# k-sheridan/mantis

Measured on AMD Instinct MI355X. Metric: poses/sec + p50 per-frame latency, 1280x720 4-cam batch, higher is better.
Workload: dtype f64; 1 GPU; config3: 4-cam 1280x720 rig, shared map, full mantis3 path per camera + joint rig Gauss-Newton; cams_per_rig=4, contexts_per_gpu=6, landmarks=720, parallelism=rig-data-parallel x1

## Files before the change

include/mantis.h:

```cpp
#ifndef MANTIS_H
#define MANTIS_H
#include <stddef.h>
#include <stdint.h>

#ifdef __cplusplus
extern "C" {
#endif

#define MANTIS_ABI_VERSION 5

typedef enum mantis_status {
  MANTIS_OK = 0,
  MANTIS_ERR_ARG = 1,
  MANTIS_ERR_DEVICE = 2,
  MANTIS_ERR_OOM = 3,
  MANTIS_ERR_CAPACITY = 4,
  MANTIS_ERR_STATE = 5,
  MANTIS_ERR_COMM = 6
} mantis_status;

typedef enum mantis_reason {
  MANTIS_PUBLISHED = 0,
  MANTIS_NO_QUADS = 1,
  MANTIS_NO_HYPS = 2,
// ... 147 lines not shown
mantis_status mantis_gn_accumulate(void* ctx, const double* T_w_b, const double* T_base_cam, int32_t n_cams,
                                   const double* obs, int32_t n_obs, double* acc28);
mantis_status mantis_gn_solve(const double* acc28, double lambda, double* T_w_b, double* delta6);

mantis_status mantis_comm_unique_id(void* id128);
mantis_status mantis_comm_init(void* ctx, const void* id128, int32_t nranks, int32_t rank);
mantis_status mantis_comm_info(void* ctx, int32_t* nranks, int32_t* rank);
mantis_status mantis_gn_allreduce(void* ctx, double* acc28);

typedef struct mantis_synth_cam {
  double fx, fy, cx, cy;
  double k[4];
  double R_wc[9];
  double pos[3];
  int32_t w, h;
  int32_t pad[2];
} mantis_synth_cam;
mantis_status mantis_synth_render(void* ctx, const mantis_synth_cam* cams, int32_t n, const uint64_t* seeds,
                                  uint8_t* out_dev);
mantis_status mantis_device_alloc(void* ctx, size_t bytes, void** dev_ptr);
mantis_status mantis_device_free(void* ctx, void* dev_ptr);
mantis_status mantis_memcpy_h2d(void* ctx, void* dst_dev, const void* src_host, size_t bytes);
mantis_status mantis_memcpy_d2h(void* ctx, void* dst_host, const void* src_dev, size_t bytes);
mantis_status mantis_synchronize(void* ctx);
int32_t mantis_kernel_times(void* ctx, const char** names, float* ms, int32_t max);
mantis_status mantis_set_profiling(void* ctx, int32_t on);

size_t mantis_frame_debug_size(void);
mantis_status mantis_get_frame_debug(void* ctx, int32_t frame, void* out, size_t bytes);
mantis_status mantis_get_contours(void* ctx, int32_t frame, int32_t* counts, int32_t* holes, int32_t max_borders,
                                  int32_t* points, int32_t max_points, int32_t* n_borders);
int32_t mantis_frame_counters(void* ctx, int32_t frame, int32_t* out, int32_t max);
int32_t mantis_small_batch_frames(void* ctx);

typedef struct mantis_track_params {
  int32_t struct_size;
  int32_t particles;
  int32_t iterations;
  double sigma_rot, sigma_t;
  int32_t min_projections;
  int32_t record;
  double max_error;
} mantis_track_params;
void mantis_default_track_params(void* ctx , mantis_track_params* p);

typedef struct mantis_track_result {
  int32_t status, tracked, n_proj, n_scored;
  double T_w_b[16];
  double error, seed_error;
  double iter_err[11];
  int32_t iter_pick[10];
  uint64_t rng_state_after;
} mantis_track_result;
void mantis_track_sizes(int32_t* params_bytes, int32_t* result_bytes);

mantis_status mantis_track_batch(void* ctx, const mantis_image* cams, int32_t n_rigs, int32_t cams_per_rig,
                                 const double* T_w_b_pred, const mantis_track_params* p, mantis_track_result* out);
mantis_status mantis_track(void* ctx, const mantis_image* cams, int32_t n_cams, const mantis_motion* motion,
                           const mantis_track_params* p, mantis_result* out, mantis_track_result* tout);
mantis_status mantis_get_track_record(void* ctx, int32_t rig, int32_t iteration, double* T_w_b, double* c2w,
                                      int64_t* sums, int32_t* counts, int32_t* n_particles);

#define MANTIS_MCL_TAU_DEFAULT 63478.0
typedef struct mantis_mcl_params {
  int32_t struct_size;
  int32_t n_particles;
// ... 334 lines not shown
```

mantis_amd/__init__.py:

```python
import ctypes as C
import os

import numpy as np

ROOT = os.path.dirname(os.path.dirname(os.path.abspath(__file__)))
LIB_PATH = os.environ.get("MANTIS_AMD_LIB") or os.path.join(os.path.dirname(os.path.abspath(__file__)),
                                                             "libmantis_amd.so")

MANTIS_OK = 0
REASONS = {0: "published", 1: "no_quads", 2: "no_hyps", 3: "yaw_ambiguous", 4: "no_yaw"}


class MantisConfig(C.Structure):
    _fields_ = [("struct_size", C.c_int32), ("device", C.c_int32), ("max_cams", C.c_int32),
                ("max_width", C.c_int32), ("max_height", C.c_int32), ("rng_seed", C.c_uint64),
                ("canny_low", C.c_int32), ("polygon_epsilon", C.c_int32),
                ("search_radius_multiplier", C.c_double), ("grid_spacing", C.c_double),
                ("particles", C.c_int32), ("iterations", C.c_int32), ("gn_enable", C.c_int32),
                ("gn_iterations", C.c_int32), ("max_quads", C.c_int32), ("max_contour_points", C.c_int32),
                ("quad_gn_iterations", C.c_int32), ("rig_weighting", C.c_int32)]


class MantisImage(C.Structure):
    _fields_ = [("width", C.c_int32), ("height", C.c_int32), ("step_bytes", C.c_int32), ("mem_kind", C.c_int32),
# ... 196 lines not shown
        ("shift_err", C.c_double * 81), ("top20_err", C.c_double * 20), ("yaw_err", C.c_double * 4),
        ("yaw_best", C.c_int32), ("min_yaw_diff", C.c_double), ("pub_c2w", C.c_double * 12),
        ("pub_error", C.c_double), ("position", C.c_double * 3), ("orientation_xyzw", C.c_double * 4),
        ("covariance", C.c_double * 36), ("rng_state_after", C.c_uint64), ("n_scored", C.c_int32),
    ]


_lib = None

_SIGS = {
    "mantis_abi_version": (C.c_int32, []),
    "mantis_default_config": (None, [C.POINTER(MantisConfig)]),
    "mantis_create": (C.c_int, [C.POINTER(MantisConfig), C.POINTER(C.c_void_p)]),
    "mantis_destroy": (C.c_int, [C.c_void_p]),
    "mantis_last_error": (C.c_char_p, [C.c_void_p]),
    "mantis_set_map": (C.c_int, [C.c_void_p, C.c_void_p, C.c_int32, C.c_void_p, C.c_int32, C.c_void_p, C.c_int32]),
    "mantis_parse_coordinates": (C.c_int32, [C.c_char_p, C.c_void_p, C.c_int32]),
    "mantis_rng_get": (C.c_int, [C.c_void_p, C.POINTER(C.c_uint64)]),
    "mantis_rng_set": (C.c_int, [C.c_void_p, C.c_uint64]),
    "mantis_process": (C.c_int, [C.c_void_p, C.POINTER(MantisImage), C.c_int32, C.POINTER(MantisMotion),
                                 C.POINTER(MantisResult), C.POINTER(MantisCamResult)]),
    "mantis_process_batch": (C.c_int, [C.c_void_p, C.POINTER(MantisImage), C.c_int32, C.c_int32,
                                       C.POINTER(MantisResult), C.POINTER(MantisCamResult)]),
    "mantis_canny": (C.c_int, [C.c_void_p, C.POINTER(MantisImage), C.c_void_p]),
    "mantis_hysteresis": (C.c_int, [C.c_void_p, C.c_void_p, C.c_int32, C.c_int32, C.c_void_p]),
    "mantis_masks": (C.c_int, [C.c_void_p, C.POINTER(MantisImage), C.c_void_p, C.c_void_p]),
    "mantis_detect_quads": (C.c_int, [C.c_void_p, C.POINTER(MantisImage), C.c_void_p, C.c_int32,
                                      C.POINTER(C.c_int32)]),
    "mantis_score_hypotheses": (C.c_int, [C.c_void_p, C.POINTER(MantisImage), C.c_void_p, C.c_void_p, C.c_int32,
                                          C.c_int32, C.c_void_p, C.c_void_p]),
    "mantis_rpp_batch": (C.c_int, [C.c_void_p, C.c_void_p, C.c_void_p, C.c_int32, C.c_void_p, C.c_void_p,
                                   C.c_void_p, C.c_void_p]),
    "mantis_small_batch_frames": (C.c_int32, [C.c_void_p]),
    "mantis_rpp_solve": (C.c_int, [C.c_void_p, C.c_void_p, C.c_void_p, C.c_int32, C.c_int32, C.c_void_p,
                                   C.c_void_p, C.c_void_p, C.c_void_p, C.c_void_p]),
    "mantis_quad_gn": (C.c_int, [C.c_void_p, C.c_void_p, C.c_void_p, C.c_int32, C.c_void_p, C.c_void_p, C.c_int32,
                                 C.c_void_p, C.c_void_p]),
    "mantis_get_rig_weights": (C.c_int, [C.c_void_p, C.c_int32, C.c_void_p, C.c_void_p, C.c_void_p,
                                         C.POINTER(C.c_int32)]),
    "mantis_markov_init": (C.c_int, [C.c_void_p, C.c_int32, C.c_void_p]),
    "mantis_markov_sense": (C.c_int, [C.c_void_p, C.c_void_p, C.c_void_p]),
    "mantis_markov_convolve": (C.c_int, [C.c_void_p, C.c_void_p, C.c_void_p, C.c_void_p]),
    "mantis_markov_weight": (C.c_int, [C.c_void_p, C.c_int32, C.c_void_p, C.c_int32, C.c_void_p]),
    "mantis_markov_get": (C.c_int, [C.c_void_p, C.c_void_p, C.c_void_p, C.c_void_p]),
    "mantis_set_prior_pose": (C.c_int, [C.c_void_p, C.c_void_p]),
    "mantis_get_prior_pose": (C.c_int, [C.c_void_p, C.c_void_p, C.POINTER(C.c_int32)]),
    "mantis_synth_render": (C.c_int, [C.c_void_p, C.POINTER(SynthCamC), C.c_int32, C.c_void_p, C.c_void_p]),
    "mantis_device_alloc": (C.c_int, [C.c_void_p, C.c_size_t, C.POINTER(C.c_void_p)]),
    "mantis_device_free": (C.c_int, [C.c_void_p, C.c_void_p]),
    "mantis_memcpy_h2d": (C.c_int, [C.c_void_p, C.c_void_p, C.c_void_p, C.c_size_t]),
    "mantis_memcpy_d2h": (C.c_int, [C.c_void_p, C.c_void_p, C.c_void_p, C.c_size_t]),
    "mantis_synchronize": (C.c_int, [C.c_void_p]),
    "mantis_kernel_times": (C.c_int32, [C.c_void_p, C.POINTER(C.c_char_p), C.POINTER(C.c_float), C.c_int32]),
    "mantis_set_profiling": (C.c_int, [C.c_void_p, C.c_int32]),
    "mantis_frame_debug_size": (C.c_size_t, []),
    "mantis_get_frame_debug": (C.c_int, [C.c_void_p, C.c_int32, C.c_void_p, C.c_size_t]),
    "mantis_get_contours": (C.c_int, [C.c_void_p, C.c_int32, C.c_void_p, C.c_void_p, C.c_int32, C.c_void_p, C.c_int32,
                                      C.c_void_p]),
    "mantis_frame_counters": (C.c_int32, [C.c_void_p, C.c_int32, C.c_void_p, C.c_int32]),
    "mantis_gn_accumulate": (C.c_int, [C.c_void_p, C.c_void_p, C.c_void_p, C.c_int32, C.c_void_p, C.c_int32,
                                       C.c_void_p]),
    "mantis_gn_solve": (C.c_int, [C.c_void_p, C.c_double, C.c_void_p, C.c_void_p]),
    "mantis_comm_unique_id": (C.c_int, [C.c_void_p]),
    "mantis_comm_init": (C.c_int, [C.c_void_p, C.c_void_p, C.c_int32, C.c_int32]),
    "mantis_comm_info": (C.c_int, [C.c_void_p, C.POINTER(C.c_int32), C.POINTER(C.c_int32)]),
    "mantis_process_rig_sharded": (C.c_int, [C.c_void_p, C.POINTER(MantisImage), C.c_int32, C.c_int32, C.c_void_p,
# ... 1148 lines not shown
```

mantis_amd/csrc/api.hip:

```cpp
#include <hip/hip_runtime.h>
#ifndef MK_FC_THREADS
#define MK_FC_THREADS 256
#endif

#include <algorithm>
#include <atomic>
#include <cfloat>
#include <chrono>
#include <cmath>
#include <cstdio>
#include <cstdlib>
#include <cstring>
#include <mutex>
#include <sstream>
#include <string>
#include <thread>
#include <vector>

#include <rccl/rccl.h>

#include "hostbuf.h"
#include "kernels.hip"

namespace mk {
// ... 99 lines not shown
using PinBuf = Buf<T, PinAlloc>;

struct CtxStreams {
  hipStream_t s = nullptr;
  hipStream_t s_copy = nullptr;
  hipEvent_t ev_gauss = nullptr;
  hipEvent_t ev_wait = nullptr;
  std::vector<hipEvent_t> ev;
  CtxStreams() = default;
  CtxStreams(const CtxStreams&) = delete;
  CtxStreams& operator=(const CtxStreams&) = delete;
  ~CtxStreams() {
    for (hipEvent_t e : ev) (void)hipEventDestroy(e);
    if (ev_gauss) (void)hipEventDestroy(ev_gauss);
    if (ev_wait) (void)hipEventDestroy(ev_wait);
    if (s_copy) (void)hipStreamDestroy(s_copy);
    if (s) (void)hipStreamDestroy(s);
  }
};

struct Ctx : CtxStreams {
  mantis_config cfg{};
  int spin_frames = 16;
  std::string err;
  uint64_t rng_state = 1;
  DevBuf<double> d_lm;
  int nw = 0, nr = 0, ng = 0;
  int F = 0, Wmax = 0, Hmax = 0;
  int n_cu = 256;
  bool trace_lds_ok = false;
  size_t trace_lds_max = 0;
  int trace_lds_frames = 0;
  int fc_small_frames = 0;
  size_t plane = 0;
  int pool_cap = 0;
  DevBuf<uint16_t> d_lroot;
  size_t lstride = 0;
  size_t fstride = 0;
  DevBuf<uint8_t> d_bgr, d_strong, d_edge, d_det, d_mask;
  DevBuf<int32_t> d_lab;
  DevBuf<uint32_t> d_eb, d_b1, d_b2;
  DevBuf<uint32_t> d_mbits;
  size_t bstride = 0;
  int morph_bh = 48;
  int morph_walk = 1 << 20;
  bool runs_done = false;
  int morph_walk_small = 48;
  size_t pf_mask_lds = 0;
  int hyst_epoch = 3;
  bool hyst_rec = true;
  size_t hyst_rec_lds = 0;
  bool pf_split = true;
  DevBuf<uint32_t> d_dbits;
  DevBuf<uint32_t> d_tbits;
  size_t tstride = 0;
  DevBuf<int32_t> d_rowb;
  size_t rstride = 0;
  size_t dstride = 0;
  DevBuf<FrameDesc> d_frames;
  DevBuf<Border> d_borders;
  DevBuf<int32_t> d_bcount, d_boff, d_pool, d_scratch;
  DevBuf<QuadRec> d_quads;
  DevBuf<RppOut> d_rpp;
  DevBuf<RppItem> d_items;
  DevBuf<rpp::Refine> d_refine;
  DevBuf<int32_t> d_jobs0, d_jobs1;
// ... 415 lines not shown
  const int Wp = W + 2, Hp = H + 2;
  dim3 grow((Hp + 4 * RUN_RPW - 1) / (4 * RUN_RPW), n);
  uint16_t* rx = c->d_lroot;
  if (!c->runs_done) {
    k_run_count<<<grow, 256, 0, c->s>>>(c->d_dbits, c->dstride, c->d_rowb, c->rstride, Wp, Hp);
    k_run_scan<<<n, 256, 0, c->s>>>(c->d_rowb, c->rstride, c->d_st, Hp);
    k_run_emit<<<grow, 256, 0, c->s>>>(c->d_dbits, c->dstride, c->d_rowb, c->rstride, rx, c->d_lab, P, Wp, Hp);
  }
  k_run_band<<<dim3((Hp + RB_ROWS - 1) / RB_ROWS, n), RB_THREADS, 0, c->s>>>(c->d_rowb, c->rstride, rx, c->d_lab, P, Wp, Hp);
  const int seams = (Hp - 1) / RB_ROWS;
  if (seams > 0)
    k_run_seam<<<dim3((seams + 3) / 4, n), 256, 0, c->s>>>(c->d_rowb, c->rstride, rx, c->d_lab, P, Wp, Hp);
  k_run_border<<<grow, 256, 0, c->s>>>(c->d_rowb, c->rstride, rx, c->d_lab, P, c->d_borders, c->d_st, Wp, Hp,
                                       kMaxBorders);
  mark(c, "components");
  const size_t tb_lds = (size_t)dbits_wpw(Wp) * Hp * sizeof(uint32_t);
  k_seg_plan<<<n, 256, 0, c->s>>>(c->d_dbits, c->dstride, c->d_rowb, c->rstride, rx, c->d_lab, P, c->d_borders,
                                  c->d_st, c->d_scratch, c->pool_cap, Wp, Hp, kMaxBorders, c->seg_m);
  if (trace_on_lds(c, n, Wp, Hp)) {
    k_trace_borders_lds<<<n, 1024, tb_lds, c->s>>>(c->d_dbits, c->dstride, c->d_borders, c->d_st, c->d_scratch,
                                                   c->pool_cap, Wp, Hp, kMaxBorders, c->d_rowb, c->rstride, rx, P);
  } else {
    const int wpw = dbits_wpw(Wp);
    k_tile_bits<<<dim3((Hp + 31) / 32, n), 256, kTbRows * wpw * sizeof(uint32_t), c->s>>>(
        c->d_dbits, c->dstride, c->d_tbits, c->tstride, wpw, Wp, Hp);
    k_trace_borders<<<n, 64 * MK_TB_WAVES, 0, c->s>>>(c->d_tbits, c->tstride, c->d_borders, c->d_st, c->d_scratch, c->pool_cap, Wp,
                                        kMaxBorders, c->d_rowb, c->rstride, rx, P);
  }
  k_seg_chain<<<n, 256, 0, c->s>>>(c->d_st, c->d_bcount, c->d_scratch, c->pool_cap, kMaxBorders);
  mark(c, "border_trace");
  k_frame_contours<<<n, n <= c->fc_small_frames ? 1024 : MK_FC_THREADS, 0, c->s>>>(c->d_dbits, c->dstride, c->d_borders, c->d_st, c->d_bcount, c->d_boff,
                                         c->d_pool, c->d_scratch, c->pool_cap, c->d_quads, c->d_dbg, c->d_frames, Wp,
                                         Hp, P, kMaxBorders, (double)c->cfg.polygon_epsilon,
                                         c->cfg.search_radius_multiplier, c->d_rowb, c->rstride, rx);
  mark(c, "contours_quads");
  HIP_OK(hipGetLastError());
  return MANTIS_OK;
}

std::atomic<int> g_live_ctx[64];

unsigned objpose_blocks(const Ctx* c, size_t expected_jobs) {
  size_t b = (expected_jobs + 127) / 128;
  const int live = std::max(1, g_live_ctx[c->cfg.device & 63].load());
  const size_t cap = c->rpp_blocks > 0 ? (size_t)c->rpp_blocks : (size_t)std::max(64, 3 * c->n_cu / (2 * live));
  return (unsigned)std::max<size_t>(1, std::min(b, cap));
}

constexpr int kOpMaxRounds = 16;
template <int MODE>
mantis_status run_objpose_rounds(Ctx* c, unsigned blocks, RppItem* items, rpp::Refine* rf, const int32_t* jobs,
                                 RppQueue* q, FrameState* st, int paired, int lanes = 64, int rounds = 0) {
  if (rounds <= 0) rounds = std::max(1, c->op_rounds);
  if ((size_t)blocks * 256 > (size_t)c->op_cap) blocks = (unsigned)(c->op_cap / 256);
  for (int r = 0; r < rounds; r++) {
    const int in = (r + 1) & 1, out = r & 1;
    OpRound rd;
    int32_t* ctl = c->d_octl + 2 * (MODE * kOpMaxRounds);
    rd.in = OpPool{c->d_opool[in], c->d_ojob[in], ctl + 2 * (r > 0 ? r - 1 : 0)};
    rd.out = OpPool{c->d_opool[out], c->d_ojob[out], ctl + 2 * r};
    rd.cap = c->op_cap;
    rd.first = r == 0;
    rd.last = r == rounds - 1;
    rd.spill_below = c->op_spill;
    rd.lanes = lanes;
    rd.pad = 0;
    k_objpose_q<MODE><<<blocks, 256, 0, c->s>>>(items, rf, jobs, q, st, paired, rd);
// ... 403 lines not shown
  if (cfg.max_quads != kMaxQuads) {
    g_create_err = "max_quads: the per-frame quad capacity is fixed at 256 in this build";
    return MANTIS_ERR_ARG;
  }
  int ndev = 0;
  if (hipGetDeviceCount(&ndev) != hipSuccess || ndev <= cfg.device) {
    g_create_err = "no HIP device available (libmantis_amd requires an MI355X / gfx950 GPU)";
    return MANTIS_ERR_DEVICE;
  }
  Ctx* c = new Ctx();
  c->cfg = cfg;
  c->rng_state = cfg.rng_seed ? cfg.rng_seed : 0xffffffffULL;
  if (hipSetDevice(cfg.device) != hipSuccess || hipStreamCreateWithFlags(&c->s, hipStreamNonBlocking) != hipSuccess ||
      hipStreamCreateWithFlags(&c->s_copy, hipStreamNonBlocking) != hipSuccess ||
      hipEventCreateWithFlags(&c->ev_gauss, hipEventDisableTiming) != hipSuccess ||
      hipEventCreateWithFlags(&c->ev_wait, hipEventDisableTiming | hipEventBlockingSync) != hipSuccess) {
    g_create_err = "hipSetDevice/hipStreamCreate failed";
    mantis_destroy(c);
    return MANTIS_ERR_DEVICE;
  }
  if (hipDeviceGetAttribute(&c->n_cu, hipDeviceAttributeMultiprocessorCount, cfg.device) != hipSuccess || c->n_cu < 1)
    c->n_cu = 256;
  if (const char* e = std::getenv("MANTIS_RPP_BLOCKS")) c->rpp_blocks = std::atoi(e);
  if (const char* e = std::getenv("MANTIS_OP_ROUNDS")) c->op_rounds = std::max(1, std::min(kOpMaxRounds, std::atoi(e)));
  if (const char* e = std::getenv("MANTIS_OP_SPILL")) c->op_spill = std::max(0, std::min(64, std::atoi(e)));
  if (const char* e = std::getenv("MANTIS_OP_LANES_SMALL")) c->op_lanes_small = std::max(1, std::min(64, std::atoi(e)));
  if (const char* e = std::getenv("MANTIS_OP_ROUNDS_SMALL")) c->op_rounds_small = std::max(1, std::min(kOpMaxRounds, std::atoi(e)));
  if (const char* e = std::getenv("MANTIS_SEG_M")) c->seg_m = std::max(0, std::min(4096, std::atoi(e)));
  if (const char* e = std::getenv("MANTIS_CANNY_STRIP")) c->canny_strip = c->canny_small = std::atoi(e);
  if (const char* e = std::getenv("MANTIS_CANNY_CAT")) c->canny_cat = e[0] != '0';
  if (const char* e = std::getenv("MANTIS_GN_FUSED")) c->gn_fused_all = e[0] != '0';
  if (const char* e = std::getenv("MANTIS_PF_INIT")) c->pf_init = std::max(0, std::min(2, std::atoi(e)));
  if (const char* e = std::getenv("MANTIS_HYST_REC")) c->hyst_rec = e[0] != '0';
  {
    const char* pc = std::getenv("DEBUG_CLR_GRAPH_PACKET_CAPTURE");
    c->use_graphs = pc && pc[0] == '0';
    if (const char* e = std::getenv("MANTIS_GRAPHS")) c->use_graphs = c->use_graphs && e[0] != '0';
  }
  if (const char* e = std::getenv("MANTIS_HYST_EPOCH0")) c->hyst_epoch = std::max(3, std::min(255, std::atoi(e)));
  c->F = cfg.max_cams;
  c->Wmax = cfg.max_width;
  c->Hmax = cfg.max_height;
  c->plane = (size_t)(c->Wmax + 2) * (c->Hmax + 2);
  c->bstride = bits::tiled_words(c->Wmax, c->Hmax);
  c->dstride = (size_t)dbits_wpw(c->Wmax + 2) * (c->Hmax + 2);
  c->pool_cap = cfg.max_contour_points;
  {
    c->trace_lds_max = 160 * 1024 - 512 * 8 - 64;
    c->trace_lds_ok = hipFuncSetAttribute((const void*)k_trace_borders_lds, hipFuncAttributeMaxDynamicSharedMemorySize,
                                          (int)c->trace_lds_max) == hipSuccess;
    const char* so = getenv("MANTIS_SCREEN");
    c->screen_off = so && so[0] == '0';
    const char* e = getenv("MANTIS_TRACE_LDS_FRAMES");
    c->trace_lds_frames = e ? atoi(e) : c->n_cu / 4;
    const char* e2 = getenv("MANTIS_FC_SMALL_FRAMES");
    c->fc_small_frames = e2 ? atoi(e2) : c->n_cu / 4;
    const char* e3 = getenv("MANTIS_PF_SPLIT");
    c->pf_split = !(e3 && e3[0] == '0');
  }
  {
    const size_t ml = bits::tiled_words(c->Wmax, c->Hmax) * 4;
    hipFuncAttributes a1;
    c->pf_mask_lds = 0;
    if (!getenv("MANTIS_PF_MASK_GLOBAL") &&
        hipFuncGetAttributes(&a1, (const void*)k_score_pf<kPfThreads, kPfSplit, true>) == hipSuccess &&
        a1.sharedSizeBytes + ml <= 160 * 1024 &&
// ... 858 lines not shown
  auto it = std::find(c->user_allocs.begin(), c->user_allocs.end(), dev_ptr);
  if (it == c->user_allocs.end()) return MANTIS_ERR_ARG;
  c->user_allocs.erase(it);
  HIP_OK(hipFree(dev_ptr));
  return MANTIS_OK;
}
mantis_status mantis_memcpy_h2d(void* ctx, void* dst, const void* src, size_t bytes) {
  Ctx* c = (Ctx*)ctx;
  if (c) bind_device(c);
  if (!c) return MANTIS_ERR_ARG;
  HIP_OK(hipMemcpyAsync(dst, src, bytes, hipMemcpyHostToDevice, c->s));
  HIP_OK(hipStreamSynchronize(c->s));
  return MANTIS_OK;
}
mantis_status mantis_memcpy_d2h(void* ctx, void* dst, const void* src, size_t bytes) {
  Ctx* c = (Ctx*)ctx;
  if (c) bind_device(c);
  if (!c) return MANTIS_ERR_ARG;
  HIP_OK(hipMemcpyAsync(dst, src, bytes, hipMemcpyDeviceToHost, c->s));
  HIP_OK(hipStreamSynchronize(c->s));
  return MANTIS_OK;
}
mantis_status mantis_synchronize(void* ctx) {
  Ctx* c = (Ctx*)ctx;
  if (c) bind_device(c);
  if (!c) return MANTIS_ERR_ARG;
  HIP_OK(hipStreamSynchronize(c->s));
  return MANTIS_OK;
}
int32_t mantis_small_batch_frames(void* ctx) {
  const Ctx* c = (const Ctx*)ctx;
  return c ? c->fc_small_frames : -1;
}
int32_t mantis_kernel_times(void* ctx, const char** names, float* ms, int32_t max) {
  Ctx* c = (Ctx*)ctx;
  if (c) bind_device(c);
  if (!c) return 0;
  int n = (int)c->last_ms.size();
  for (int i = 0; i < n && i < max; i++) {
    if (names) names[i] = c->last_names[i].c_str();
    if (ms) ms[i] = c->last_ms[i];
  }
  return n;
}
mantis_status mantis_set_profiling(void* ctx, int32_t on) {
  Ctx* c = (Ctx*)ctx;
  if (c) bind_device(c);
  if (!c) return MANTIS_ERR_ARG;
  c->prof = on != 0;
  return MANTIS_OK;
}

}

#include "gn_impl.hip"
#include "dense_impl.hip"
#include "markov_impl.hip"
#include "track_impl.hip"
#include "mcl_impl.hip"
#include "mcl_modes_impl.hip"
#include "mcl_color_impl.hip"
#include "refine_impl.hip"
#include "smooth_impl.hip"
#include "lag_impl.hip"
#include "linecal_impl.hip"
#include "mcl_refine_impl.hip"
// ... 2 lines not shown
```

mantis_amd/csrc/kernels.hip:

```cpp
#include <hip/hip_runtime.h>

#include <cfloat>
#include <cstdint>
#include <type_traits>

#include "mk_bits.h"
#include "mk_contour.h"
#include "mk_gn.h"
#include "mk_math.h"
#include "mk_rpp.h"
#include "mk_shard.h"
#include "mk_sort.h"
#include "mk_track.h"
#include "mk_types.h"
#include "synth.h"

namespace mk {

#ifndef MK_DPP_SCAN
#define MK_DPP_SCAN 1
#endif
__device__ inline int wave_incl_scan(int v, int lane) {
#if MK_DPP_SCAN
  (void)lane;
// ... 1918 lines not shown
      bx[j] = j == i ? px : bx[j];
      by[j] = j == i ? py : by[j];
#endif
    }
    k++;
    if ((k & 7) == 0) store8(k - 8);
#else
    ((uint32_t*)chunks)[(size_t)cur * kChunk + k] = (uint32_t)px | ((uint32_t)py << 16);
    k++;
#endif
  }
  __device__ void flush() {
    if (cur < 0) return;
#if MK_CHUNK_BUF
    if (k & 7) store8(k & ~7);
#endif
    ccount[cur] = k;
  }
};

__device__ inline void wave_argmax(double& d, int& idx) {
  for (int o = 32; o > 0; o >>= 1) {
    const double d2 = __shfl_xor(d, o);
    const int i2 = __shfl_xor(idx, o);
    if (d2 > d || (d2 == d && i2 < idx)) { d = d2; idx = i2; }
  }
}

typedef __attribute__((address_space(3))) int32_t lds_i32;
#ifndef MK_WAVE_STK
#define MK_WAVE_STK 14
#endif
constexpr int kWaveStk = MK_WAVE_STK;
template <class STK>
__device__ int approx_poly_wave(const uint32_t* __restrict__ src, int count, double eps, int32_t* dst, STK stk,
                                int max_dp, int cap = 0x7fffffff) {
  const int lane = threadIdx.x & 63;
  if (count == 0) return 0;
  eps *= eps;
  int top = 0, nc = 0, rs_s = 0, pos = 0;
  bool le_eps = false;
  int spx = 0, spy = 0;
  for (int it = 0; it < 3; it++) {
    pos = (pos + rs_s) % count;
    spx = PtPacked::x(src[pos]);
    spy = PtPacked::y(src[pos]);
    double best = 0;
    int bj = 0x7fffffff;
    for (int j = 1 + lane; j < count; j += 64) {
      int q = pos + j;
      if (q >= count) q -= count;
      const uint32_t v = src[q];
      const double dx = PtPacked::x(v) - spx, dy = PtPacked::y(v) - spy;
      const double d = dx * dx + dy * dy;
      if (d > best) { best = d; bj = j; }
    }
    wave_argmax(best, bj);
    if (best > 0) rs_s = bj;
    le_eps = best <= eps;
  }
  if (!le_eps) {
    const int sl_s = pos % count, sl_e = (rs_s + sl_s) % count;
    if (lane == 0) {
      stk[0] = sl_e; stk[1] = sl_s;
      stk[2] = sl_s; stk[3] = sl_e;
    }
    top = 2;
  } else {
// ... 29 lines not shown
    } else {
      le_eps = true;
    }
    if (le_eps) {
      if (lane == 0) { dst[2 * nc] = spx; dst[2 * nc + 1] = spy; }
      nc++;
      if (max_dp > 0 && nc >= max_dp) return max_dp + 1;
    } else {
      if (top + 2 > cap) return -1;
      if (lane == 0) {
        stk[2 * top] = rs_s; stk[2 * top + 1] = sl_e;
        stk[2 * top + 2] = sl_s; stk[2 * top + 3] = rs_s;
      }
      top += 2;
    }
  }
  int r = 0;
  if (lane == 0) r = approx_cleanup(dst, nc, eps, true);
  return __shfl(r, 0);
}

__device__ inline bool ccomp_before(int pa, int ha, int ka, int pb, int hb, int kb) {
  if (pa != pb) return pa > pb;
  if (ha != hb) return ha < hb;
  return ka > kb;
}

#ifndef MK_LONG_BORDER
#define MK_LONG_BORDER 128
#endif
constexpr int kLongBorder = MK_LONG_BORDER;
static_assert(kLongBorder <= 128, "k_frame_contours' length buckets (count / 4) hold counts up to 128");
constexpr int kMaxLong = 512;

struct RawQuad {
  int32_t c[8];
  int32_t parent, hole, key;
};

constexpr int kTbRows = 34;
__device__ __host__ inline int tb_groups(int Wp) { return ((Wp - 2) >> 4) + 1; }
__device__ __host__ inline size_t tbits_words(int Wp, int Hp) {
  return (size_t)tb_groups(Wp) * kTbRows * (size_t)((Hp + 31) >> 5);
}
__device__ inline uint32_t tb_off(int x, int y, int G) {
  return (uint32_t)(((y >> 5) * G + (x >> 4)) * kTbRows + (y & 31));
}
__global__ __launch_bounds__(256) void k_tile_bits(const uint32_t* __restrict__ dbits, size_t dstride,
                                                   uint32_t* __restrict__ tbits, size_t tstride, int wpw, int Wp,
                                                   int Hp) {
  extern __shared__ uint32_t tl_band[];
  const int f = blockIdx.y, ty = blockIdx.x, t = threadIdx.x;
  const uint32_t* src = dbits + (size_t)f * dstride;
  const int r0 = 32 * ty - 1;
  for (int i = t; i < kTbRows * wpw; i += 256) {
    const int e = i / wpw, r = r0 + e;
    tl_band[i] = r >= 0 && r < Hp ? src[(size_t)r * wpw + (i - e * wpw)] : 0u;
  }
  __syncthreads();
  const int G = tb_groups(Wp);
  uint32_t* dst = tbits + (size_t)f * tstride + (size_t)ty * G * kTbRows;
  for (int o = t; o < G * kTbRows; o += 256) {
    const int g = o / kTbRows, e = o - g * kTbRows;
    const int p = 16 * g - 8, w = p >> 5, sh = p & 31;
    const uint32_t lo = w >= 0 ? tl_band[e * wpw + w] : 0u, hi = w + 1 < wpw ? tl_band[e * wpw + w + 1] : 0u;
    dst[o] = (lo >> sh) | (hi << (32 - sh));
// ... 486 lines not shown
  for (;;) {
    int j = 0;
    j = atomicAdd(&next_job, 1);
    if (j >= NS) break;
    const int sd = T.sdir[j];
    if (sd == kSegUnused || sd == kSegAlias) continue;
    const Border b = bs[T.border[j]];
    ChunkEmit em{chunks, owner, ordv, ordv + max_chunks, &st[f].n_chunks, max_chunks, j, -1, 0, 0, false};
    int steps = 0, nx = -1;
    if (sd == kSegSingle) {
      const uint32_t p = (uint32_t)T.pos[j];
      em((int)(p & 0xffffu) - 1, (int)(p >> 16) - 1);
      em.n_pts = 1;
    } else {
      nx = walk_segment_lds(nbh, next_lut, em, b, Wp, (uint32_t)T.pos[j], sd, M, r, X, T.rowbase, steps);
    }
    T.cnt[j] = em.n_pts;
    T.next[j] = nx;
    em.flush();
    if (em.ovf) atomicOr(&st[f].overflow, 2);
    atomicMax(&st[f].trace_steps_max, steps);
  }
}

#ifndef MK_FC_CPL
#define MK_FC_CPL 2
#endif
#ifndef MK_FC_CU
#define MK_FC_CU 8
#endif
#ifndef MK_FC_WPE
#define MK_FC_WPE 5
#endif
__global__ __launch_bounds__(1024) __attribute__((amdgpu_waves_per_eu(MK_FC_WPE))) void k_frame_contours(const uint32_t* __restrict__ dbits, size_t dstride,
                                                         const Border* __restrict__ borders,
                                                         FrameState* st, int32_t* __restrict__ counts,
                                                         int32_t* __restrict__ offs, int32_t* __restrict__ pool,
                                                         int32_t* __restrict__ scratch, int pool_cap,
                                                         QuadRec* __restrict__ quads, FrameDebug* dbg,
                                                         const FrameDesc* __restrict__ frames, int Wp, int Hp,
                                                         size_t plane, int border_cap, double eps, double search_mult,
                                                         const int32_t* __restrict__ rowb, size_t rstride,
                                                         const uint16_t* __restrict__ rx) {
  __shared__ int32_t scan[1024];
  __shared__ RawQuad raw[kMaxQuads];
  __shared__ int32_t nraw, total, nkeep;
  __shared__ int32_t idx4[kMaxQuads][4];
  __shared__ int32_t nbr[kMaxQuads];
  __shared__ int32_t kpos[kMaxQuads];
  __shared__ int32_t ord[kMaxQuads];
  __shared__ float qcx[kMaxQuads], qcy[kMaxQuads];
  __shared__ double qside[kMaxQuads];
  __shared__ int32_t nchunk, nlong;
  __shared__ int32_t longs[kMaxLong];
  const int f = blockIdx.x;
  const int tid = threadIdx.x;
  const uint32_t* B = dbits + (size_t)f * dstride;
  const int wpw = dbits_wpw(Wp);
  const Border* bs = borders + (size_t)f * border_cap;
  int32_t* cnt = counts + (size_t)f * border_cap;
  int32_t* off = offs + (size_t)f * border_cap;
  uint32_t* pl = (uint32_t*)(pool + 2 * (size_t)f * pool_cap);
  int32_t* sc = scratch + 4 * (size_t)f * pool_cap;
  int nb = st[f].n_borders;
  if (nb > border_cap) nb = border_cap;
  auto emit_raw = [&](int i, const int32_t* q4) {
    const int q = atomicAdd(&nraw, 1);
    if (q < kMaxQuads) {
      for (int k = 0; k < 8; k++) raw[q].c[k] = q4[k];
      int par = bs[i].parent;
      if (par < 0) {
        const int pr = -par - 1;
        par = run_at_row(rowb + (size_t)f * rstride, Hp, pr) * Wp + rx[(size_t)f * plane + pr];
      }
      raw[q].parent = par;
      raw[q].hole = bs[i].hole;
      raw[q].key = bs[i].key;
    } else {
      atomicOr(&st[f].overflow, 4);
    }
  };
  const uint64_t t0 = wall_clock64();
#ifdef MK_HYST_TICKS
#define MK_TICK(k)
#else
// ... 81 lines not shown
  if (tid < 33) hist[tid] = 0;
  if (tid == 0) { next_long = 0; next_short = 0; }
  __syncthreads();
  bool sorted = nb <= 1024;
  if (sorted) {
    for (int i = tid; i < nb; i += blockDim.x) {
      const int c = cnt[i];
      if (c > kLongBorder) {
        const int k = atomicAdd(&nlong, 1);
        if (k < kMaxLong) longs[k] = i;
      } else {
        atomicAdd(&hist[c >> 2], 1);
      }
    }
    __syncthreads();
    sorted = nlong <= kMaxLong;
    if (sorted) {
      if (tid == 0) {
        int acc = 0;
        for (int b = 32; b >= 0; b--) {
          const int h = hist[b];
          hist[b] = acc;
          acc += h;
        }
        nshort = acc;
      }
      __syncthreads();
      for (int i = tid; i < nb; i += blockDim.x) {
        const int c = cnt[i];
        if (c <= kLongBorder) scan[atomicAdd(&hist[c >> 2], 1)] = i;
      }
      __syncthreads();
      const int lane = tid & 63;
      for (;;) {
        int k = 0;
        if (lane == 0) k = atomicAdd(&next_long, 1);
        k = __shfl(k, 0);
        if (k >= nlong) break;
        const int i = longs[k], o = off[i], c = cnt[i];
        int32_t* dst = sc + 4 * (size_t)o;
        int32_t* stk = dst + 2 * (size_t)c;
        int m = approx_poly_wave(pl + o, c, eps, dst, (lds_i32*)wstk[tid >> 6], 10, kWaveStk);
        if (m < 0) m = approx_poly_wave(pl + o, c, eps, dst, stk, 10);
        if (m == 4 && lane == 0) emit_raw(i, dst);
      }
#ifdef MK_FC_TICK_SPLIT
      MK_TICK(2);
#endif
      for (;;) {
        int k = 0;
        if (lane == 0) k = atomicAdd(&next_short, 64);
        k = __shfl(k, 0);
        if (k >= nshort) break;
        if (k + lane < nshort) {
          const int i = scan[k + lane], o = off[i], c = cnt[i];
          int32_t* dst = sc + 4 * (size_t)o;
          int32_t* stk = dst + 2 * (size_t)c;
          const int m = approx_poly(PtPacked{pl + o}, c, eps, true, dst, stk, 10);
          if (m == 4) emit_raw(i, dst);
        }
      }
      __syncthreads();
#ifdef MK_FC_TICK_SPLIT
      MK_TICK(3);
#else
      MK_TICK(2);
#endif
    } else {
      __syncthreads();
      if (tid == 0) nlong = 0;
      __syncthreads();
    }
  }
  if (!sorted) {
    for (int i = tid; i < nb; i += blockDim.x) {
      const int o = off[i], c = cnt[i];
      if (c > kLongBorder) {
        const int k = atomicAdd(&nlong, 1);
        if (k < kMaxLong) { longs[k] = i; continue; }
      }
      int32_t* dst = sc + 4 * (size_t)o;
      int32_t* stk = dst + 2 * (size_t)c;
      int m = approx_poly(PtPacked{pl + o}, c, eps, true, dst, stk, 10);
      if (m == 4) emit_raw(i, dst);
    }
    __syncthreads();
    MK_TICK(2);
    {
      const int wave = tid >> 6, nwaves = blockDim.x >> 6;
      const int nl = nlong < kMaxLong ? nlong : kMaxLong;
      for (int k = wave; k < nl; k += nwaves) {
        const int i = longs[k], o = off[i], c = cnt[i];
        int32_t* dst = sc + 4 * (size_t)o;
        int32_t* stk = dst + 2 * (size_t)c;
        const int m = approx_poly_wave(pl + o, c, eps, dst, stk, 10);
        if (m == 4 && (tid & 63) == 0) emit_raw(i, dst);
      }
    }
  }
  __syncthreads();
#ifndef MK_FC_TICK_SPLIT
  MK_TICK(3);
#endif
  const int nq = nraw < kMaxQuads ? nraw : kMaxQuads;
  for (int i = tid; i < nq; i += blockDim.x) {
    int r = 0;
    for (int j = 0; j < nq; j++)
      if (ccomp_before(raw[j].parent, raw[j].hole, raw[j].key, raw[i].parent, raw[i].hole, raw[i].key)) r++;
    ord[r] = i;
  }
  __syncthreads();
  for (int r = tid; r < nq; r += blockDim.x) {
    const RawQuad& q = raw[ord[r]];
    int dx = q.c[0] - q.c[2], dy = q.c[1] - q.c[3];
    qside[r] = sqrt((double)(dx * dx + dy * dy));
    float xs = 0, ys = 0;
    for (int k = 0; k < 4; k++) { xs += (float)q.c[2 * k]; ys += (float)q.c[2 * k + 1]; }
    qcx[r] = xs / (float)4;
    qcy[r] = ys / (float)4;
  }
  __syncthreads();
  for (int i = tid; i < nq; i += blockDim.x) {
    float radius = (float)(search_mult * qside[i]);
    float bd[4] = {0, 0, 0, 0};
    int bi[4] = {0, 0, 0, 0};
    int nh = 0;
    for (int j = 0; j < nq; j++) {
      float d0 = qcx[j] - qcx[i], d1 = qcy[j] - qcy[i];
// ... 2007 lines not shown
```

Measured before the change: 30400 rig poses/s.

## Stage contour points into reused LDS before polygon approximation

The filter-stage shared arrays are overlaid in a union with a staging buffer. During the sorted polygon-approximation phase, each wave copies its border's packed contour points from global memory into its own LDS region and runs approx_poly / approx_poly_wave on the LDS copy. This is done for both long borders (per wave) and short borders (per lane, packed with a wave prefix scan). The aim is to cut repeated global reads of contour points, at the cost of an extra copy pass and wave barriers. An env knob and an info query entry point are added.

```diff
diff --git a/include/mantis.h b/include/mantis.h
--- a/include/mantis.h
+++ b/include/mantis.h
@@ -203,6 +203,7 @@
                                   int32_t* points, int32_t max_points, int32_t* n_borders);
 int32_t mantis_frame_counters(void* ctx, int32_t frame, int32_t* out, int32_t max);
 int32_t mantis_small_batch_frames(void* ctx);
+int32_t mantis_contour_stage_info(void* ctx, int32_t* out, int32_t max);
 
 typedef struct mantis_track_params {
   int32_t struct_size;
diff --git a/mantis_amd/__init__.py b/mantis_amd/__init__.py
--- a/mantis_amd/__init__.py
+++ b/mantis_amd/__init__.py
@@ -252,6 +252,7 @@
     "mantis_rpp_batch": (C.c_int, [C.c_void_p, C.c_void_p, C.c_void_p, C.c_int32, C.c_void_p, C.c_void_p,
                                    C.c_void_p, C.c_void_p]),
     "mantis_small_batch_frames": (C.c_int32, [C.c_void_p]),
+    "mantis_contour_stage_info": (C.c_int32, [C.c_void_p, C.c_void_p, C.c_int32]),
     "mantis_rpp_solve": (C.c_int, [C.c_void_p, C.c_void_p, C.c_void_p, C.c_int32, C.c_int32, C.c_void_p,
                                    C.c_void_p, C.c_void_p, C.c_void_p, C.c_void_p]),
     "mantis_quad_gn": (C.c_int, [C.c_void_p, C.c_void_p, C.c_void_p, C.c_int32, C.c_void_p, C.c_void_p, C.c_int32,
diff --git a/mantis_amd/csrc/api.hip b/mantis_amd/csrc/api.hip
--- a/mantis_amd/csrc/api.hip
+++ b/mantis_amd/csrc/api.hip
@@ -155,6 +155,7 @@
   size_t trace_lds_max = 0;
   int trace_lds_frames = 0;
   int fc_small_frames = 0;
+  bool fc_stage = true;
   size_t plane = 0;
   int pool_cap = 0;
   DevBuf<uint16_t> d_lroot;
@@ -636,7 +637,7 @@
   k_frame_contours<<<n, n <= c->fc_small_frames ? 1024 : MK_FC_THREADS, 0, c->s>>>(c->d_dbits, c->dstride, c->d_borders, c->d_st, c->d_bcount, c->d_boff,
                                          c->d_pool, c->d_scratch, c->pool_cap, c->d_quads, c->d_dbg, c->d_frames, Wp,
                                          Hp, P, kMaxBorders, (double)c->cfg.polygon_epsilon,
-                                         c->cfg.search_radius_multiplier, c->d_rowb, c->rstride, rx);
+                                         c->cfg.search_radius_multiplier, c->d_rowb, c->rstride, rx, c->fc_stage ? 1 : 0);
   mark(c, "contours_quads");
   HIP_OK(hipGetLastError());
   return MANTIS_OK;
@@ -1106,6 +1107,7 @@
   if (const char* e = std::getenv("MANTIS_GN_FUSED")) c->gn_fused_all = e[0] != '0';
   if (const char* e = std::getenv("MANTIS_PF_INIT")) c->pf_init = std::max(0, std::min(2, std::atoi(e)));
   if (const char* e = std::getenv("MANTIS_HYST_REC")) c->hyst_rec = e[0] != '0';
+  if (const char* e = std::getenv("MANTIS_FC_STAGE")) c->fc_stage = e[0] != '0';
   {
     const char* pc = std::getenv("DEBUG_CLR_GRAPH_PACKET_CAPTURE");
     c->use_graphs = pc && pc[0] == '0';
@@ -2030,6 +2032,14 @@
   const Ctx* c = (const Ctx*)ctx;
   return c ? c->fc_small_frames : -1;
 }
+int32_t mantis_contour_stage_info(void* ctx, int32_t* out, int32_t max) {
+  const Ctx* c = (const Ctx*)ctx;
+  if (!c || !out) return -1;
+  const int32_t v[6] = {c->fc_stage ? 1 : 0, kLongBorder, kFcStageWords, MK_FC_THREADS, kWaveStk, kMaxLong};
+  int n = 0;
+  for (; n < 6 && n < max; n++) out[n] = v[n];
+  return n;
+}
 int32_t mantis_kernel_times(void* ctx, const char** names, float* ms, int32_t max) {
   Ctx* c = (Ctx*)ctx;
   if (c) bind_device(c);
diff --git a/mantis_amd/csrc/kernels.hip b/mantis_amd/csrc/kernels.hip
--- a/mantis_amd/csrc/kernels.hip
+++ b/mantis_amd/csrc/kernels.hip
@@ -1974,8 +1974,9 @@
 #define MK_WAVE_STK 14
 #endif
 constexpr int kWaveStk = MK_WAVE_STK;
-template <class STK>
-__device__ int approx_poly_wave(const uint32_t* __restrict__ src, int count, double eps, int32_t* dst, STK stk,
+typedef __attribute__((address_space(3))) uint32_t lds_u32;
+template <class SRC, class STK>
+__device__ int approx_poly_wave(SRC __restrict__ src, int count, double eps, int32_t* dst, STK stk,
                                 int max_dp, int cap = 0x7fffffff) {
   const int lane = threadIdx.x & 63;
   if (count == 0) return 0;
@@ -2071,6 +2072,16 @@
 constexpr int kLongBorder = MK_LONG_BORDER;
 static_assert(kLongBorder <= 128, "k_frame_contours' length buckets (count / 4) hold counts up to 128");
 constexpr int kMaxLong = 512;
+constexpr int kFcStageWords = 11 * kMaxQuads;
+
+struct PtLds {
+  const lds_u32* p;
+  static constexpr int kAhead = PtPacked::kAhead;
+  typedef uint32_t Raw;
+  __device__ Raw ld(int i) const { return p[i]; }
+  __device__ static int x(Raw r) { return PtPacked::x(r); }
+  __device__ static int y(Raw r) { return PtPacked::y(r); }
+};
 
 struct RawQuad {
   int32_t c[8];
@@ -2623,6 +2634,9 @@
 #ifndef MK_FC_WPE
 #define MK_FC_WPE 5
 #endif
+#ifndef MK_FC_STAGE_SHORT
+#define MK_FC_STAGE_SHORT 1
+#endif
 __global__ __launch_bounds__(1024) __attribute__((amdgpu_waves_per_eu(MK_FC_WPE))) void k_frame_contours(const uint32_t* __restrict__ dbits, size_t dstride,
                                                          const Border* __restrict__ borders,
                                                          FrameState* st, int32_t* __restrict__ counts,
@@ -2632,16 +2646,29 @@
                                                          const FrameDesc* __restrict__ frames, int Wp, int Hp,
                                                          size_t plane, int border_cap, double eps, double search_mult,
                                                          const int32_t* __restrict__ rowb, size_t rstride,
-                                                         const uint16_t* __restrict__ rx) {
+                                                         const uint16_t* __restrict__ rx, int stage) {
   __shared__ int32_t scan[1024];
   __shared__ RawQuad raw[kMaxQuads];
   __shared__ int32_t nraw, total, nkeep;
-  __shared__ int32_t idx4[kMaxQuads][4];
-  __shared__ int32_t nbr[kMaxQuads];
-  __shared__ int32_t kpos[kMaxQuads];
-  __shared__ int32_t ord[kMaxQuads];
-  __shared__ float qcx[kMaxQuads], qcy[kMaxQuads];
-  __shared__ double qside[kMaxQuads];
+  struct Filter {
+    double qside[kMaxQuads];
+    int32_t idx4[kMaxQuads][4];
+    int32_t nbr[kMaxQuads], kpos[kMaxQuads], ord[kMaxQuads];
+    float qcx[kMaxQuads], qcy[kMaxQuads];
+  };
+  __shared__ union {
+    uint32_t stage[kFcStageWords];
+    Filter filter;
+  } post;
+  static_assert(sizeof(Filter) == sizeof(uint32_t) * kFcStageWords, "the filter's arrays fill the staging storage exactly");
+  static_assert(kFcStageWords % 16 == 0, "an equal region for each of 4 or 16 waves");
+  auto& qside = post.filter.qside;
+  auto& idx4 = post.filter.idx4;
+  auto& nbr = post.filter.nbr;
+  auto& kpos = post.filter.kpos;
+  auto& ord = post.filter.ord;
+  auto& qcx = post.filter.qcx;
+  auto& qcy = post.filter.qcy;
   __shared__ int32_t nchunk, nlong;
   __shared__ int32_t longs[kMaxLong];
   const int f = blockIdx.x;
@@ -2789,6 +2816,8 @@
       }
       __syncthreads();
       const int lane = tid & 63;
+      const int region = stage ? kFcStageWords / (int)(blockDim.x >> 6) : 0;
+      lds_u32* const reg = (lds_u32*)post.stage + (tid >> 6) * (kFcStageWords / (int)(blockDim.x >> 6));
       for (;;) {
         int k = 0;
         if (lane == 0) k = atomicAdd(&next_long, 1);
@@ -2797,8 +2826,27 @@
         const int i = longs[k], o = off[i], c = cnt[i];
         int32_t* dst = sc + 4 * (size_t)o;
         int32_t* stk = dst + 2 * (size_t)c;
-        int m = approx_poly_wave(pl + o, c, eps, dst, (lds_i32*)wstk[tid >> 6], 10, kWaveStk);
-        if (m < 0) m = approx_poly_wave(pl + o, c, eps, dst, stk, 10);
+        int m;
+        if (c <= region) {
+          constexpr int kU = 4;
+          for (int j0 = lane; j0 < c; j0 += 64 * kU) {
+            uint32_t v[kU];
+#pragma unroll
+            for (int u = 0; u < kU; u++) v[u] = pl[o + min(j0 + 64 * u, c - 1)];
+#pragma unroll
+            for (int u = 0; u < kU; u++)
+              if (j0 + 64 * u < c) reg[j0 + 64 * u] = v[u];
+          }
+          __builtin_amdgcn_fence(__ATOMIC_RELEASE, "wavefront");
+          __builtin_amdgcn_wave_barrier();
+          __builtin_amdgcn_fence(__ATOMIC_ACQUIRE, "wavefront");
+          m = approx_poly_wave((const lds_u32*)reg, c, eps, dst, (lds_i32*)wstk[tid >> 6], 10, kWaveStk);
+          if (m < 0) m = approx_poly_wave((const lds_u32*)reg, c, eps, dst, stk, 10);
+          __builtin_amdgcn_wave_barrier();
+        } else {
+          m = approx_poly_wave((const uint32_t*)(pl + o), c, eps, dst, (lds_i32*)wstk[tid >> 6], 10, kWaveStk);
+          if (m < 0) m = approx_poly_wave((const uint32_t*)(pl + o), c, eps, dst, stk, 10);
+        }
         if (m == 4 && lane == 0) emit_raw(i, dst);
       }
 #ifdef MK_FC_TICK_SPLIT
@@ -2809,10 +2857,30 @@
         if (lane == 0) k = atomicAdd(&next_short, 64);
         k = __shfl(k, 0);
         if (k >= nshort) break;
-        if (k + lane < nshort) {
-          const int i = scan[k + lane], o = off[i], c = cnt[i];
-          int32_t* dst = sc + 4 * (size_t)o;
-          int32_t* stk = dst + 2 * (size_t)c;
+        const bool on = k + lane < nshort;
+        const int i = on ? scan[k + lane] : 0;
+        const int o = on ? off[i] : 0, c = on ? cnt[i] : 0;
+        int32_t* dst = sc + 4 * (size_t)o;
+        int32_t* stk = dst + 2 * (size_t)c;
+        const int sregion = MK_FC_STAGE_SHORT ? region : 0;
+        const int inc = sregion ? wave_incl_scan(c, lane) : 0;
+        if (sregion && __shfl(inc, 63) <= sregion) {
+          lds_u32* const mine = reg + (inc - c);
+          constexpr int kU = 8;
+          for (int j0 = 0; __any(j0 < c); j0 += kU) {
+            uint32_t v[kU];
+#pragma unroll
+            for (int u = 0; u < kU; u++) v[u] = pl[o + max(min(j0 + u, c - 1), 0)];
+#pragma unroll
+            for (int u = 0; u < kU; u++)
+              if (j0 + u < c) mine[j0 + u] = v[u];
+          }
+          if (on) {
+            const int m = approx_poly(PtLds{mine}, c, eps, true, dst, stk, 10);
+            if (m == 4) emit_raw(i, dst);
+          }
+          __builtin_amdgcn_wave_barrier();
+        } else if (on) {
           const int m = approx_poly(PtPacked{pl + o}, c, eps, true, dst, stk, 10);
           if (m == 4) emit_raw(i, dst);
         }
@@ -2850,7 +2918,7 @@
         const int i = longs[k], o = off[i], c = cnt[i];
         int32_t* dst = sc + 4 * (size_t)o;
         int32_t* stk = dst + 2 * (size_t)c;
-        const int m = approx_poly_wave(pl + o, c, eps, dst, stk, 10);
+        const int m = approx_poly_wave((const uint32_t*)(pl + o), c, eps, dst, stk, 10);
         if (m == 4 && (tid & 63) == 0) emit_raw(i, dst);
       }
     }
```

Measured after the change: 30730 rig poses/s, median of 4. Within noise of the previous version (+1.1%).
